# PaddlePaddle/PaddleScience

Measured on NVIDIA H100. Metric: collocation-points/sec PDE residual loss+grad (LDC N-S), higher is better.
Workload: dtype f32

## Files before the change

### paddlescience_b200/csrc/kernels_wgmma.cuh

```cuda
#pragma once

#include "kernels_thin.cuh"

#ifndef PPSCI_EMUL
#include <stdint.h>

namespace ppsci {
namespace wg {

constexpr int KCH = 32;
constexpr int THREADS = 256;
constexpr int TM = 64;
constexpr int A_TILE_BYTES = TM * KCH * 4;
__host__ __device__ inline int tile_points(int C) { return TM / C; }

__host__ __device__ inline int stage_bytes(int N) { return 2 * A_TILE_BYTES + 2 * N * KCH * 4; }
__host__ __device__ inline int fwd_smem_bytes(int N) { return 2 * stage_bytes(N) + 1024 + 64; }
constexpr int PREFETCH_MAX_CS = 8;

__host__ __device__ __forceinline__ uint32_t sw128(int row, int kk) {
  return (uint32_t)(row * 128 + ((((kk >> 2) ^ row) & 7) << 4) + ((kk & 3) << 2));
}
__device__ __forceinline__ uint32_t sw128_q(int row, int kq) { return (uint32_t)(row * 128 + (((kq ^ row) & 7) << 4)); }

__device__ __forceinline__ uint32_t smem_u32(const void* p) { return (uint32_t)__cvta_generic_to_shared(p); }

__device__ __forceinline__ float tf32_rn(float x) {
  uint32_t u;
  asm("cvt.rna.tf32.f32 %0, %1;" : "=r"(u) : "f"(x));
  return __uint_as_float(u);
}

__device__ __forceinline__ void mbar_init(uint32_t bar, uint32_t count) {
  asm volatile("mbarrier.init.shared::cta.b64 [%0], %1;" ::"r"(bar), "r"(count) : "memory");
}
__device__ __forceinline__ void mbar_expect_tx(uint32_t bar, uint32_t bytes) {
  asm volatile("mbarrier.arrive.expect_tx.shared::cta.b64 _, [%0], %1;" ::"r"(bar), "r"(bytes) : "memory");
}
__device__ __forceinline__ bool mbar_try_wait(uint32_t bar, uint32_t parity) {
  uint32_t ok;
  asm volatile(
      "{\n\t.reg .pred p;\n\t"
      "mbarrier.try_wait.parity.shared::cta.b64 p, [%1], %2;\n\t"
      "selp.u32 %0, 1, 0, p;\n\t}"
      : "=r"(ok)
      : "r"(bar), "r"(parity)
      : "memory");
  return ok != 0;
}
__device__ __forceinline__ void mbar_wait(uint32_t bar, uint32_t parity) {
  uint32_t spins = 0;
  while (!mbar_try_wait(bar, parity)) {
    if (++spins > (1u << 26)) __trap();
  }
}
__device__ __forceinline__ void bulk_g2s(uint32_t dst_smem, const void* src, uint32_t bytes, uint32_t bar) {
  asm volatile("cp.async.bulk.shared::cluster.global.mbarrier::complete_tx::bytes [%0], [%1], %2, [%3];" ::"r"(dst_smem),
               "l"(src), "r"(bytes), "r"(bar)
               : "memory");
}
__device__ __forceinline__ void fence_proxy_async() { asm volatile("fence.proxy.async.shared::cta;" ::: "memory"); }

__device__ __forceinline__ uint64_t make_desc(uint32_t saddr) {
  uint64_t d = 0;
  d |= (uint64_t)((saddr & 0x3FFFFu) >> 4);
  d |= (uint64_t)1 << 16;
  d |= (uint64_t)(1024 >> 4) << 32;
  d |= (uint64_t)1 << 62;
  return d;
}
__device__ __forceinline__ void wgmma_fence() { asm volatile("wgmma.fence.sync.aligned;" ::: "memory"); }
__device__ __forceinline__ void wgmma_commit() { asm volatile("wgmma.commit_group.sync.aligned;" ::: "memory"); }
template <int N>
__device__ __forceinline__ void wgmma_wait() {
  asm volatile("wgmma.wait_group.sync.aligned %0;" ::"n"(N) : "memory");
}
#define WG_T0 "%0, %1, %2, %3, %4, %5, %6, %7"
#define WG_T1 WG_T0 ", %8, %9, %10, %11, %12, %13, %14, %15"
#define WG_T2 WG_T1 ", %16, %17, %18, %19, %20, %21, %22, %23"
#define WG_T3 WG_T2 ", %24, %25, %26, %27, %28, %29, %30, %31"
#define WG_T4 WG_T3 ", %32, %33, %34, %35, %36, %37, %38, %39"
#define WG_T5 WG_T4 ", %40, %41, %42, %43, %44, %45, %46, %47"
#define WG_T6 WG_T5 ", %48, %49, %50, %51, %52, %53, %54, %55"
#define WG_T7 WG_T6 ", %56, %57, %58, %59, %60, %61, %62, %63"
#define WG_O8(b) "+f"(d[b]), "+f"(d[b + 1]), "+f"(d[b + 2]), "+f"(d[b + 3]), "+f"(d[b + 4]), "+f"(d[b + 5]), "+f"(d[b + 6]), "+f"(d[b + 7])
#define WG_O0 WG_O8(0)
#define WG_O1 WG_O0, WG_O8(8)
#define WG_O2 WG_O1, WG_O8(16)
#define WG_O3 WG_O2, WG_O8(24)
#define WG_O4 WG_O3, WG_O8(32)
#define WG_O5 WG_O4, WG_O8(40)
#define WG_O6 WG_O5, WG_O8(48)
#define WG_O7 WG_O6, WG_O8(56)
#define WG_MMA(M, G, IA, IB, IP)                                                                                  \
  __device__ __forceinline__ void wgmma_tf32(float (&d)[M / 2], uint64_t da, uint64_t db, uint32_t accumulate) { \
    asm volatile(                                                                                                 \
        "{\n\t.reg .pred p;\n\t"                                                                                  \
        "setp.ne.b32 p, %" #IP ", 0;\n\t"                                                                          \
        "wgmma.mma_async.sync.aligned.m64n" #M "k8.f32.tf32.tf32 {" WG_T##G "}, %" #IA ", %" #IB ", p, 1, 1;\n\t}"  \
        : WG_O##G                                                                                                 \
        : "l"(da), "l"(db), "r"(accumulate));                                                                     \
  }
WG_MMA(16, 0, 8, 9, 10)
WG_MMA(32, 1, 16, 17, 18)
WG_MMA(48, 2, 24, 25, 26)
WG_MMA(64, 3, 32, 33, 34)
WG_MMA(80, 4, 40, 41, 42)
WG_MMA(96, 5, 48, 49, 50)
WG_MMA(112, 6, 56, 57, 58)
WG_MMA(128, 7, 64, 65, 66)
#undef WG_MMA

__global__ void k_wg_prep_w(const float* __restrict__ W, float* __restrict__ img, int K, int N, int transposed) {
  const long long i = (long long)blockIdx.x * blockDim.x + threadIdx.x;
  if (i >= (long long)K * N) return;
  const int n = (int)(i / K), k = (int)(i % K);
  const float w = transposed ? W[(long long)n * K + k] : W[(long long)k * N + n];
  const float hi = tf32_rn(w);
  float* blk = img + (long long)(k / KCH) * 2 * N * KCH;
  const uint32_t off = sw128(n, k % KCH) >> 2;
  blk[off] = hi;
  blk[(long long)N * KCH + off] = w - hi;
}

struct WgArgs {
  AOperand<float> A;
  JetLayout J;
  const float* Wimg;
  int Kdim;
  int Kvalid;
  int Nout;
  const float* bias;
  float* Out;
  int ldo;
  long long oplane;
  long long Np;
  int num_tiles;
  const float* Zprev;
  int ldz;
  long long zplane;
  int act;
};

__device__ __forceinline__ unsigned char* xchg(unsigned char* base_ptr, int sbytes, int N, int r, int col) {
  return base_ptr + sbytes + 2 * A_TILE_BYTES + r * N * 4 + ((((col >> 2) ^ r) & 7) << 4) + (((col >> 2) & ~7) << 4) +
         (col & 3) * 4;
}

template <class L, int NQ, bool DX>
__global__ void __launch_bounds__(THREADS, 1) k_wg_layer(WgArgs g) {
  PPSCI_DYN_SMEM(smem_dyn);
  const uint32_t base = (smem_u32(smem_dyn) + 1023u) & ~1023u;
  unsigned char* base_ptr = smem_dyn + (base - smem_u32(smem_dyn));
  constexpr int CS = L::CS;
  constexpr int TP = TM / CS;
  constexpr int rows_used = CS * TP;
  constexpr int PPR = (THREADS / 32) * 4;
  constexpr int MAXI = (TP + PPR - 1) / PPR;
  constexpr int N = NQ * 32;
  constexpr int NH = N / 2;
  constexpr bool PREFETCH = CS <= PREFETCH_MAX_CS;
  const int sbytes = stage_bytes(N);
  const uint32_t bar0 = base + 2 * sbytes;
  const uint32_t b_bytes = (uint32_t)(2 * N * KCH * 4);
  const int tid = threadIdx.x, warp = tid >> 5, lane = tid & 31, wgi = tid >> 7;
  const int kq = lane & 7, psub = lane >> 3;
  const int nchunks = g.Kdim / KCH;
  const int act = g.A.act;

  if (tid == 0) {
    mbar_init(bar0, 1);
    mbar_init(bar0 + 8, 1);
    asm volatile("fence.mbarrier_init.release.cluster;" ::: "memory");
  }
  for (int s = 0; s < 2; ++s) {
    float4* az = reinterpret_cast<float4*>(base_ptr + s * sbytes);
    for (int i = tid; i < 2 * A_TILE_BYTES / 16; i += THREADS) az[i] = make_float4(0.f, 0.f, 0.f, 0.f);
  }
  fence_proxy_async();
  __syncthreads();

  float4 z[MAXI][CS];
  bool zok[MAXI];
  auto load_z = [&](int tile, int j) {
#pragma unroll
    for (int i = 0; i < MAXI; ++i) {
      const int pl = warp * 4 + psub + i * PPR;
      const long long p = (long long)tile * TP + pl;
      zok[i] = pl < TP && tile < g.num_tiles && p < g.Np;
      if (g.Kvalid && j * KCH + 4 * kq >= g.Kvalid) zok[i] = false;
      const float* src = g.A.Z + p * g.A.ld + j * KCH + 4 * kq;
#pragma unroll
      for (int c = 0; c < CS; ++c)
        z[i][c] = zok[i] ? __ldg(reinterpret_cast<const float4*>(src + (long long)c * g.A.plane)) : make_float4(0.f, 0.f, 0.f, 0.f);
    }
  };
  if constexpr (PREFETCH) load_z(blockIdx.x, 0);

  float ex[NH / 2], cr[NH / 2];
  const int rbase = (warp & 3) * 16 + (lane >> 2);
  const int cbase = wgi * NH + 2 * (lane & 3);
  uint32_t it = 0;
  for (int tile = blockIdx.x; tile < g.num_tiles; tile += gridDim.x) {
    const long long p0 = (long long)tile * TP;
#pragma unroll
    for (int e = 0; e < NH / 2; ++e) ex[e] = cr[e] = 0.f;
    for (int j = 0; j < nchunks; ++j, ++it) {
      const uint32_t s = it & 1u;
      wgmma_wait<1>();
      __syncthreads();
      const uint32_t st_addr = base + s * sbytes;
      unsigned char* st_ptr = base_ptr + s * sbytes;
      if (tid == 0) {
        mbar_expect_tx(bar0 + 8 * s, b_bytes);
        bulk_g2s(st_addr + 2 * A_TILE_BYTES, g.Wimg + (long long)j * 2 * N * KCH, b_bytes, bar0 + 8 * s);
      }
      if constexpr (!PREFETCH) load_z(tile, j);
#pragma unroll
      for (int i = 0; i < MAXI; ++i) {
        const int pl = warp * 4 + psub + i * PPR;
        if (pl >= TP) continue;
        const bool valid = zok[i];
        float yout[CS][4];
        if constexpr (DX) {
#pragma unroll
          for (int c = 0; c < CS; ++c) {
            yout[c][0] = z[i][c].x; yout[c][1] = z[i][c].y; yout[c][2] = z[i][c].z; yout[c][3] = z[i][c].w;
          }
        } else {
#pragma unroll
          for (int t = 0; t < 4; ++t) {
            auto comp = [&](const float4& v) { return t == 0 ? v.x : t == 1 ? v.y : t == 2 ? v.z : v.w; };
            float sc[6];
            float y0;
            act_coef<float, L::KM>(act, comp(z[i][0]), y0, sc);
            yout[0][t] = valid ? y0 : 0.f;
            jet_fwd<float, L>(g.J, sc, [&](int c) { return comp(z[i][c]); }, [&](int c, float v) { yout[c][t] = valid ? v : 0.f; });
          }
        }
#pragma unroll
        for (int c = 0; c < CS; ++c) {
          float4 h, l;
          h.x = tf32_rn(yout[c][0]); h.y = tf32_rn(yout[c][1]); h.z = tf32_rn(yout[c][2]); h.w = tf32_rn(yout[c][3]);
          l.x = yout[c][0] - h.x; l.y = yout[c][1] - h.y; l.z = yout[c][2] - h.z; l.w = yout[c][3] - h.w;
          const uint32_t off = sw128_q(c * TP + pl, kq);
          *reinterpret_cast<float4*>(st_ptr + off) = h;
          *reinterpret_cast<float4*>(st_ptr + A_TILE_BYTES + off) = l;
        }
      }
      if constexpr (PREFETCH) {
        if (j + 1 < nchunks) load_z(tile, j + 1);
        else load_z(tile + gridDim.x, 0);
      }
      fence_proxy_async();
      __syncthreads();
      mbar_wait(bar0 + 8 * s, (it >> 1) & 1u);
      const uint64_t a_hi = make_desc(st_addr), a_lo = make_desc(st_addr + A_TILE_BYTES);
      const uint64_t b_hi = make_desc(st_addr + 2 * A_TILE_BYTES + wgi * NH * 128), b_lo = b_hi + (uint64_t)(N * 128 / 16);
      wgmma_fence();
#pragma unroll
      for (int ks = 0; ks < KCH / 8; ++ks) {
        const uint64_t inc = (uint64_t)(2 * ks);
        const uint32_t first = (j == 0 && ks == 0) ? 0u : 1u;
        wgmma_tf32(ex, a_hi + inc, b_hi + inc, first);
        wgmma_tf32(cr, a_lo + inc, b_hi + inc, first);
        wgmma_tf32(cr, a_hi + inc, b_lo + inc, 1u);
      }
      wgmma_commit();
    }
    wgmma_wait<0>();
    if constexpr (!DX) {
#pragma unroll
      for (int h = 0; h < 2; ++h) {
        const int r = rbase + 8 * h;
        const int c = r / TP, pl = r - c * TP;
        const long long p = p0 + pl;
        if (r >= rows_used || p >= g.Np) continue;
        float* out_row = g.Out + (long long)c * g.oplane + p * g.ldo;
#pragma unroll
        for (int j = 0; j < NH / 8; ++j) {
          const int col = cbase + 8 * j;
          float2 v = make_float2(ex[4 * j + 2 * h] + cr[4 * j + 2 * h], ex[4 * j + 2 * h + 1] + cr[4 * j + 2 * h + 1]);
          if (c == 0 && g.bias) {
            v.x += __ldg(g.bias + col);
            v.y += __ldg(g.bias + col + 1);
          }
          *reinterpret_cast<float2*>(out_row + col) = v;
        }
      }
    } else {
      __syncthreads();
#pragma unroll
      for (int h = 0; h < 2; ++h) {
        const int r = rbase + 8 * h;
#pragma unroll
        for (int j = 0; j < NH / 8; ++j)
          *reinterpret_cast<float2*>(xchg(base_ptr, sbytes, N, r, cbase + 8 * j)) =
              make_float2(ex[4 * j + 2 * h] + cr[4 * j + 2 * h], ex[4 * j + 2 * h + 1] + cr[4 * j + 2 * h + 1]);
      }
      constexpr int N4 = N / 4;
      auto load_zc = [&](int item, float4 (&zc)[CS]) {
        const int pl = item / N4, q = item - pl * N4;
        const long long p = p0 + pl;
        if (item >= TP * N4 || p >= g.Np) return;
#pragma unroll
        for (int c = 0; c < CS; ++c)
          zc[c] = __ldg(reinterpret_cast<const float4*>(g.Zprev + (long long)c * g.zplane + p * g.ldz + 4 * q));
      };
      float4 znext[CS];
      if constexpr (PREFETCH) load_zc(tid, znext);
      __syncthreads();
      for (int item = tid; item < TP * N4; item += THREADS) {
        const int pl = item / N4, q = item - pl * N4;
        const long long p = p0 + pl;
        float4 zc[CS];
        if constexpr (PREFETCH) {
#pragma unroll
          for (int c = 0; c < CS; ++c) zc[c] = znext[c];
          load_zc(item + THREADS, znext);
        } else {
          load_zc(item, zc);
        }
        if (p >= g.Np) continue;
        float4 xc[CS];
#pragma unroll
        for (int c = 0; c < CS; ++c) xc[c] = *reinterpret_cast<const float4*>(xchg(base_ptr, sbytes, N, c * TP + pl, 4 * q));
        float ob[CS][4];
#pragma unroll
        for (int t = 0; t < 4; ++t) {
          auto comp = [&](const float4& v) { return t == 0 ? v.x : t == 1 ? v.y : t == 2 ? v.z : v.w; };
          float sc[6];
          float y0;
          act_coef<float, L::KM + 1>(g.act, comp(zc[0]), y0, sc);
          ob[0][t] = jet_adj<float, L>(g.J, sc, [&](int c) { return comp(zc[c]); }, [&](int c) { return comp(xc[c]); },
                                       [&](int c, float v) { ob[c][t] = v; });
        }
        float* out = g.Out + p * g.ldo + 4 * q;
#pragma unroll
        for (int c = 0; c < CS; ++c)
          *reinterpret_cast<float4*>(out + (long long)c * g.oplane) = make_float4(ob[c][0], ob[c][1], ob[c][2], ob[c][3]);
      }
      fence_proxy_async();
      __syncthreads();
    }
  }
}

__host__ __device__ constexpr int dw_pch(int C) { return C >= 8 ? 4 : C >= 3 ? 8 : 32 / C; }
__host__ __device__ constexpr int dw_groups(int C) { return dw_pch(C) / 4 * C; }
__host__ __device__ constexpr int dw_ksteps(int C) { return (dw_groups(C) + 1) / 2; }
__host__ __device__ constexpr int dw_atoms(int C) { return (dw_ksteps(C) + 3) / 4; }
__host__ __device__ constexpr int dw_maxq(int C) { return C <= 5 ? 4 : C <= 8 ? 2 : 1; }
__host__ __device__ constexpr int dw_smem_bytes(int C, int bnq) {
  return 2 * 2 * dw_atoms(C) * bnq * 32 * 128 + bnq * 32 * 4 + dw_pch(C) / 4 * 2 * C * 256 * 4 + bnq * 32 * 2 * 256 + 1024;
}
constexpr int DW_TK = 128;
constexpr int DW_FLUSH_ROWS = 512;
__host__ __device__ constexpr int dw_flush(int C) {
  return DW_FLUSH_ROWS / (dw_pch(C) * C) > 1 ? DW_FLUSH_ROWS / (dw_pch(C) * C) : 1;
}

struct WgDwArgs {
  AOperand<float> A;
  JetLayout J;
  const float* Zbar;
  int ldzb;
  long long zbplane;
  int Kdim;
  int Nout;
  int col_blocks;
  float* dW;
  float* db;
  long long Np;
  int chunks_per_split;
};

__device__ __forceinline__ void wgmma_tf32_rA_m64n64(float (&d)[32], const uint32_t (&a)[4], uint64_t db) {
  asm volatile(
      "{\n\t.reg .pred p;\n\t"
      "setp.ne.b32 p, %37, 0;\n\t"
      "wgmma.mma_async.sync.aligned.m64n64k8.f32.tf32.tf32 "
      "{%0, %1, %2, %3, %4, %5, %6, %7, %8, %9, %10, %11, %12, %13, %14, %15, "
      "%16, %17, %18, %19, %20, %21, %22, %23, %24, %25, %26, %27, %28, %29, %30, %31}, "
      "{%32, %33, %34, %35}, %36, p, 1, 1;\n\t}"
      : "+f"(d[0]), "+f"(d[1]), "+f"(d[2]), "+f"(d[3]), "+f"(d[4]), "+f"(d[5]), "+f"(d[6]), "+f"(d[7]), "+f"(d[8]),
        "+f"(d[9]), "+f"(d[10]), "+f"(d[11]), "+f"(d[12]), "+f"(d[13]), "+f"(d[14]), "+f"(d[15]), "+f"(d[16]),
        "+f"(d[17]), "+f"(d[18]), "+f"(d[19]), "+f"(d[20]), "+f"(d[21]), "+f"(d[22]), "+f"(d[23]), "+f"(d[24]),
        "+f"(d[25]), "+f"(d[26]), "+f"(d[27]), "+f"(d[28]), "+f"(d[29]), "+f"(d[30]), "+f"(d[31])
      : "r"(a[0]), "r"(a[1]), "r"(a[2]), "r"(a[3]), "l"(db), "r"(1u));
}
__device__ __forceinline__ void wgmma_tf32_rA_m64n32(float (&d)[16], const uint32_t (&a)[4], uint64_t db) {
  asm volatile(
      "{\n\t.reg .pred p;\n\t"
      "setp.ne.b32 p, %21, 0;\n\t"
      "wgmma.mma_async.sync.aligned.m64n32k8.f32.tf32.tf32 "
      "{%0, %1, %2, %3, %4, %5, %6, %7, %8, %9, %10, %11, %12, %13, %14, %15}, "
      "{%16, %17, %18, %19}, %20, p, 1, 1;\n\t}"
      : "+f"(d[0]), "+f"(d[1]), "+f"(d[2]), "+f"(d[3]), "+f"(d[4]), "+f"(d[5]), "+f"(d[6]), "+f"(d[7]), "+f"(d[8]),
        "+f"(d[9]), "+f"(d[10]), "+f"(d[11]), "+f"(d[12]), "+f"(d[13]), "+f"(d[14]), "+f"(d[15])
      : "r"(a[0]), "r"(a[1]), "r"(a[2]), "r"(a[3]), "l"(db), "r"(1u));
}

template <class L, int BNQ>
__global__ void __launch_bounds__(THREADS, 1) k_wg_dw(WgDwArgs g) {
  PPSCI_DYN_SMEM(smem_dyn);
  const uint32_t base = (smem_u32(smem_dyn) + 1023u) & ~1023u;
  unsigned char* base_ptr = smem_dyn + (base - smem_u32(smem_dyn));
  constexpr int CS = L::CS, PCH = dw_pch(CS), QPC = PCH / 4, G = dw_groups(CS), KS = dw_ksteps(CS), NA = dw_atoms(CS);
  constexpr int BN = BNQ * 32, NB = BNQ / 2, TAIL = BNQ & 1;
  constexpr int ATOM = BN * 128;
  constexpr int STAGE = 2 * NA * ATOM;
  constexpr int BI = (G * BN + THREADS - 1) / THREADS;
  const int tid = threadIdx.x, warp = tid >> 5, lane = tid & 31, wgi = tid >> 7, t = lane & 3;
  const int kb = blockIdx.x / g.col_blocks, n0 = (blockIdx.x - kb * g.col_blocks) * BN;
  const int Np = (int)g.Np;
  const int total_chunks = (Np + PCH - 1) / PCH;
  const int ch_begin = blockIdx.y * g.chunks_per_split;
  const int ch_end = ch_begin + g.chunks_per_split < total_chunks ? ch_begin + g.chunks_per_split : total_chunks;
  if (ch_begin >= ch_end) return;
  const int act = g.A.act;
  const int krow = kb * DW_TK + wgi * 64 + (warp & 3) * 16 + (lane >> 2);

  float* bsum = reinterpret_cast<float*>(base_ptr + 2 * STAGE);
  for (int i = tid; i < (2 * STAGE + BN * 4) / 16; i += THREADS)
    reinterpret_cast<float4*>(base_ptr)[i] = make_float4(0.f, 0.f, 0.f, 0.f);
  __syncthreads();

  float ex[NB > 0 ? NB : 1][32], ext[TAIL ? 16 : 1], cr[NB > 0 ? NB : 1][32], crt[TAIL ? 16 : 1];
#pragma unroll
  for (int nb = 0; nb < NB; ++nb)
#pragma unroll
    for (int i = 0; i < 32; ++i) ex[nb][i] = cr[nb][i] = 0.f;
#pragma unroll
  for (int i = 0; i < (TAIL ? 16 : 1); ++i) ext[i] = crt[i] = 0.f;

  auto acc_at = [&](int e) -> float {
    return e < 32 * NB ? ex[e >> 5][e & 31] + cr[e >> 5][e & 31] : ext[e - 32 * NB] + crt[e - 32 * NB];
  };
  float4* part = reinterpret_cast<float4*>(base_ptr + 2 * STAGE + BN * 4 + QPC * 2 * CS * THREADS * 4);
#pragma unroll
  for (int q = 0; q < BN / 8; ++q) part[q * THREADS + tid] = make_float4(0.f, 0.f, 0.f, 0.f);
  auto flush = [&]() {
#pragma unroll
    for (int q = 0; q < BN / 8; ++q) {
      float4 p = part[q * THREADS + tid];
      p.x += acc_at(4 * q); p.y += acc_at(4 * q + 1); p.z += acc_at(4 * q + 2); p.w += acc_at(4 * q + 3);
      part[q * THREADS + tid] = p;
    }
#pragma unroll
    for (int nb = 0; nb < NB; ++nb)
#pragma unroll
      for (int i = 0; i < 32; ++i) ex[nb][i] = cr[nb][i] = 0.f;
#pragma unroll
    for (int i = 0; i < (TAIL ? 16 : 1); ++i) ext[i] = crt[i] = 0.f;
  };

  float* za = reinterpret_cast<float*>(base_ptr + 2 * STAGE + BN * 4);
  auto za_at = [&](int qq, int h, int c) -> float* { return za + ((qq * 2 + h) * CS + c) * THREADS + tid; };
  float4 zb[BI];
  auto load_a = [&](int ch) {
    const int p0 = ch * PCH;
#pragma unroll
    for (int qq = 0; qq < QPC; ++qq)
#pragma unroll
      for (int h = 0; h < 2; ++h) {
        const int p = p0 + 4 * qq + t;
        const int k = krow + 8 * h;
        const bool ok = p < Np && k < g.Kdim;
        const float* src = g.A.Z + (ok ? (long long)p * g.A.ld + k : 0);
#pragma unroll
        for (int c = 0; c < CS; ++c)
          asm volatile("cp.async.ca.shared.global [%0], [%1], 4, %2;" ::"r"(smem_u32(za_at(qq, h, c))),
                       "l"(src + (ok ? (long long)c * g.A.plane : 0)), "r"(ok ? 4 : 0)
                       : "memory");
      }
    asm volatile("cp.async.commit_group;" ::: "memory");
  };
  auto load_b = [&](int ch) {
    const int p0 = ch * PCH;
#pragma unroll
    for (int i = 0; i < BI; ++i) {
      const int item = tid + THREADS * i;
      const int gi = item / BN, n = item - gi * BN;
      const int qq = gi / CS, c = gi - qq * CS;
      const int p = p0 + 4 * qq;
      const bool ok = item < G * BN && n0 + n < g.Nout;
      const float* src = g.Zbar + (long long)c * g.zbplane + (long long)p * g.ldzb + n0 + n;
      zb[i].x = ok && p < Np ? __ldg(src) : 0.f;
      zb[i].y = ok && p + 1 < Np ? __ldg(src + g.ldzb) : 0.f;
      zb[i].z = ok && p + 2 < Np ? __ldg(src + 2 * g.ldzb) : 0.f;
      zb[i].w = ok && p + 3 < Np ? __ldg(src + 3 * g.ldzb) : 0.f;
    }
  };

  load_a(ch_begin);
  load_b(ch_begin);
  uint32_t ahi[KS][4], alo[KS][4];
  for (int ch = ch_begin; ch < ch_end; ++ch) {
    const int sidx = (ch - ch_begin) & 1;
    const uint32_t st_addr = base + sidx * STAGE;
    unsigned char* st = base_ptr + sidx * STAGE;
#pragma unroll
    for (int i = 0; i < BI; ++i) {
      const int item = tid + THREADS * i;
      if (item >= G * BN) continue;
      const int gi = item / BN, n = item - gi * BN;
      const float4 v = zb[i];
      float4 hi, lo;
      hi.x = tf32_rn(v.x); hi.y = tf32_rn(v.y); hi.z = tf32_rn(v.z); hi.w = tf32_rn(v.w);
      lo.x = v.x - hi.x; lo.y = v.y - hi.y; lo.z = v.z - hi.z; lo.w = v.w - hi.w;
      const uint32_t off = (gi >> 3) * ATOM + sw128_q(n, gi & 7);
      *reinterpret_cast<float4*>(st + off) = hi;
      *reinterpret_cast<float4*>(st + NA * ATOM + off) = lo;
      if (kb == 0 && gi % CS == 0) atomicAdd(bsum + n, (v.x + v.y) + (v.z + v.w));
    }
    wgmma_wait<0>();
    if (ch > ch_begin && (ch - ch_begin) % dw_flush(CS) == 0) flush();
    asm volatile("cp.async.wait_group 0;" ::: "memory");
    float av[QPC][2][CS];
#pragma unroll
    for (int qq = 0; qq < QPC; ++qq)
#pragma unroll
      for (int h = 0; h < 2; ++h) {
        float z[CS], sc[6];
#pragma unroll
        for (int c = 0; c < CS; ++c) z[c] = *za_at(qq, h, c);
        act_coef<float, L::KM>(act, z[0], av[qq][h][0], sc);
        jet_fwd<float, L>(g.J, sc, [&](int c) { return z[c]; }, [&](int c, float v) { av[qq][h][c] = v; });
      }
    if (ch + 1 < ch_end) load_a(ch + 1);
    fence_proxy_async();
    __syncthreads();
    if (ch + 1 < ch_end) load_b(ch + 1);
#pragma unroll
    for (int s = 0; s < KS; ++s)
#pragma unroll
      for (int e = 0; e < 2; ++e)
#pragma unroll
        for (int h = 0; h < 2; ++h) {
          const int gi = 2 * s + e;
          const float v = gi < G ? av[gi / CS][h][gi % CS] : 0.f;
          const float vh = tf32_rn(v);
          ahi[s][2 * e + h] = __float_as_uint(vh);
          alo[s][2 * e + h] = __float_as_uint(v - vh);
        }
    wgmma_fence();
#pragma unroll
    for (int s = 0; s < KS; ++s) {
      const uint64_t b_hi = make_desc(st_addr + (s >> 2) * ATOM + (s & 3) * 32);
      const uint64_t b_lo = b_hi + (uint64_t)(NA * ATOM / 16);
#pragma unroll
      for (int nb = 0; nb < NB; ++nb) {
        const uint64_t bo = (uint64_t)(nb * 64 * 128 / 16);
        wgmma_tf32_rA_m64n64(ex[nb], ahi[s], b_hi + bo);
        wgmma_tf32_rA_m64n64(cr[nb], alo[s], b_hi + bo);
        wgmma_tf32_rA_m64n64(cr[nb], ahi[s], b_lo + bo);
      }
      if constexpr (TAIL) {
        const uint64_t bo = (uint64_t)(NB * 64 * 128 / 16);
        wgmma_tf32_rA_m64n32(ext, ahi[s], b_hi + bo);
        wgmma_tf32_rA_m64n32(crt, alo[s], b_hi + bo);
        wgmma_tf32_rA_m64n32(crt, ahi[s], b_lo + bo);
      }
    }
    wgmma_commit();
  }
  wgmma_wait<0>();
#pragma unroll
  for (int h = 0; h < 2; ++h) {
    const int k = krow + 8 * h;
    if (k >= g.Kdim) continue;
    float* row = g.dW + (long long)k * g.Nout + n0;
#pragma unroll
    for (int j = 0; j < BN / 8; ++j) {
      if (n0 + 8 * j >= g.Nout) break;
      const int col = 8 * j + 2 * t;
      const float4 p = part[j * THREADS + tid];
      atomicAdd(row + col, (h ? p.z : p.x) + acc_at(4 * j + 2 * h));
      atomicAdd(row + col + 1, (h ? p.w : p.y) + acc_at(4 * j + 2 * h + 1));
    }
  }
  if (kb == 0) {
    __syncthreads();
    if (tid < BN && n0 + tid < g.Nout) atomicAdd(g.db + n0 + tid, bsum[tid]);
  }
}

}

inline int wg_kpad(int K) { return (K + wg::KCH - 1) / wg::KCH * wg::KCH; }
inline bool wg_shape_ok(int K, int N) { return K % wg::KCH == 0 && K >= 32 && K <= 1024 && N % 32 == 0 && N >= 32 && N <= 256; }
inline bool wg_plan_ok(const ppsci_plan_spec& s, const JetLayout& J) {
  return s.dtype == PPSCI_F32 && !s.gated && !act_has_param(s.act) && with_lay(WgLays{}, J, [](auto) {});
}
inline bool wg_fwd_ok(const ppsci_plan_spec& s, int l) {
  if (l == 1) return s.dense_in && s.n_layers >= 2 && s.widths[0] % 4 == 0 && wg_shape_ok(wg_kpad(s.widths[0]), s.widths[1]);
  if (l < 2 || l > s.n_layers) return false;
  return wg_shape_ok(s.widths[l - 1], s.widths[l]);
}
inline bool wg_dx_ok(const ppsci_plan_spec& s, int l) {
  if (l < 2 || l > s.n_layers) return false;
  return wg_shape_ok(s.widths[l], s.widths[l - 1]);
}

inline bool wg_dw_ok(const ppsci_plan_spec& s, int l) {
  if (l < 1 || (l == 1 && !s.dense_in) || l > s.n_layers) return false;
  const int K = s.widths[l - 1], N = s.widths[l];
  return K % 4 == 0 && N % 32 == 0 && N >= 32 && N <= 256;
}

}
#endif
```

Before: 6.042 million.

## Decouple weight B-tile staging into a 3-stage ring prefetched one chunk ahead

Splits the shared-memory stages so the A tiles stay double-buffered while the weight (B) tiles move to a separate three-slot ring with their own mbarriers. Each iteration issues the bulk copy for the next chunk (or the next tile's first chunk) ahead of time, so the weight load overlaps the current chunk's A-tile construction and wgmma instead of being issued and waited on in the same iteration. The DX exchange buffer is moved onto the last-used B slot. This uses more shared memory and adds some ring-indexing complexity, with a risk of slot-reuse hazards at tile boundaries.

```diff
diff --git a/paddlescience_b200/csrc/kernels_wgmma.cuh b/paddlescience_b200/csrc/kernels_wgmma.cuh
--- a/paddlescience_b200/csrc/kernels_wgmma.cuh
+++ b/paddlescience_b200/csrc/kernels_wgmma.cuh
@@ -14,8 +14,10 @@
 constexpr int A_TILE_BYTES = TM * KCH * 4;
 __host__ __device__ inline int tile_points(int C) { return TM / C; }
 
-__host__ __device__ inline int stage_bytes(int N) { return 2 * A_TILE_BYTES + 2 * N * KCH * 4; }
-__host__ __device__ inline int fwd_smem_bytes(int N) { return 2 * stage_bytes(N) + 1024 + 64; }
+constexpr int A_STAGE_BYTES = 2 * A_TILE_BYTES;
+constexpr int B_STAGES = 3;
+__host__ __device__ inline int b_stage_bytes(int N) { return 2 * N * KCH * 4; }
+__host__ __device__ inline int fwd_smem_bytes(int N) { return 2 * A_STAGE_BYTES + B_STAGES * b_stage_bytes(N) + 1024 + 64; }
 constexpr int PREFETCH_MAX_CS = 8;
 
 __host__ __device__ __forceinline__ uint32_t sw128(int row, int kk) {
@@ -142,9 +144,8 @@
   int act;
 };
 
-__device__ __forceinline__ unsigned char* xchg(unsigned char* base_ptr, int sbytes, int N, int r, int col) {
-  return base_ptr + sbytes + 2 * A_TILE_BYTES + r * N * 4 + ((((col >> 2) ^ r) & 7) << 4) + (((col >> 2) & ~7) << 4) +
-         (col & 3) * 4;
+__device__ __forceinline__ unsigned char* xchg(unsigned char* xb, int N, int r, int col) {
+  return xb + r * N * 4 + ((((col >> 2) ^ r) & 7) << 4) + (((col >> 2) & ~7) << 4) + (col & 3) * 4;
 }
 
 template <class L, int NQ, bool DX>
@@ -160,22 +161,21 @@
   constexpr int N = NQ * 32;
   constexpr int NH = N / 2;
   constexpr bool PREFETCH = CS <= PREFETCH_MAX_CS;
-  const int sbytes = stage_bytes(N);
-  const uint32_t bar0 = base + 2 * sbytes;
-  const uint32_t b_bytes = (uint32_t)(2 * N * KCH * 4);
+  const uint32_t b_bytes = (uint32_t)b_stage_bytes(N);
+  const uint32_t b_base = base + 2 * A_STAGE_BYTES;
+  const uint32_t bar0 = b_base + B_STAGES * b_bytes;
   const int tid = threadIdx.x, warp = tid >> 5, lane = tid & 31, wgi = tid >> 7;
   const int kq = lane & 7, psub = lane >> 3;
   const int nchunks = g.Kdim / KCH;
   const int act = g.A.act;
 
   if (tid == 0) {
-    mbar_init(bar0, 1);
-    mbar_init(bar0 + 8, 1);
+    for (int b = 0; b < B_STAGES; ++b) mbar_init(bar0 + 8 * b, 1);
     asm volatile("fence.mbarrier_init.release.cluster;" ::: "memory");
   }
   for (int s = 0; s < 2; ++s) {
-    float4* az = reinterpret_cast<float4*>(base_ptr + s * sbytes);
-    for (int i = tid; i < 2 * A_TILE_BYTES / 16; i += THREADS) az[i] = make_float4(0.f, 0.f, 0.f, 0.f);
+    float4* az = reinterpret_cast<float4*>(base_ptr + s * A_STAGE_BYTES);
+    for (int i = tid; i < A_STAGE_BYTES / 16; i += THREADS) az[i] = make_float4(0.f, 0.f, 0.f, 0.f);
   }
   fence_proxy_async();
   __syncthreads();
@@ -200,21 +200,24 @@
   float ex[NH / 2], cr[NH / 2];
   const int rbase = (warp & 3) * 16 + (lane >> 2);
   const int cbase = wgi * NH + 2 * (lane & 3);
+  auto fetch_w = [&](int j, uint32_t b) {
+    mbar_expect_tx(bar0 + 8 * b, b_bytes);
+    bulk_g2s(b_base + b * b_bytes, g.Wimg + (long long)j * 2 * N * KCH, b_bytes, bar0 + 8 * b);
+  };
+  if (tid == 0) fetch_w(0, 0);
   uint32_t it = 0;
   for (int tile = blockIdx.x; tile < g.num_tiles; tile += gridDim.x) {
     const long long p0 = (long long)tile * TP;
 #pragma unroll
     for (int e = 0; e < NH / 2; ++e) ex[e] = cr[e] = 0.f;
     for (int j = 0; j < nchunks; ++j, ++it) {
-      const uint32_t s = it & 1u;
+      const uint32_t s = it & 1u, bs = it % B_STAGES;
       wgmma_wait<1>();
       __syncthreads();
-      const uint32_t st_addr = base + s * sbytes;
-      unsigned char* st_ptr = base_ptr + s * sbytes;
-      if (tid == 0) {
-        mbar_expect_tx(bar0 + 8 * s, b_bytes);
-        bulk_g2s(st_addr + 2 * A_TILE_BYTES, g.Wimg + (long long)j * 2 * N * KCH, b_bytes, bar0 + 8 * s);
-      }
+      const uint32_t st_addr = base + s * A_STAGE_BYTES;
+      unsigned char* st_ptr = base_ptr + s * A_STAGE_BYTES;
+      if (tid == 0 && (j + 1 < nchunks || tile + (int)gridDim.x < g.num_tiles))
+        fetch_w(j + 1 < nchunks ? j + 1 : 0, bs == B_STAGES - 1 ? 0 : bs + 1);
       if constexpr (!PREFETCH) load_z(tile, j);
 #pragma unroll
       for (int i = 0; i < MAXI; ++i) {
@@ -254,9 +257,9 @@
       }
       fence_proxy_async();
       __syncthreads();
-      mbar_wait(bar0 + 8 * s, (it >> 1) & 1u);
+      mbar_wait(bar0 + 8 * bs, (it / B_STAGES) & 1u);
       const uint64_t a_hi = make_desc(st_addr), a_lo = make_desc(st_addr + A_TILE_BYTES);
-      const uint64_t b_hi = make_desc(st_addr + 2 * A_TILE_BYTES + wgi * NH * 128), b_lo = b_hi + (uint64_t)(N * 128 / 16);
+      const uint64_t b_hi = make_desc(b_base + bs * b_bytes + wgi * NH * 128), b_lo = b_hi + (uint64_t)(N * 128 / 16);
       wgmma_fence();
 #pragma unroll
       for (int ks = 0; ks < KCH / 8; ++ks) {
@@ -290,12 +293,13 @@
       }
     } else {
       __syncthreads();
+      unsigned char* xb = base_ptr + 2 * A_STAGE_BYTES + ((it - 1) % B_STAGES) * b_bytes;
 #pragma unroll
       for (int h = 0; h < 2; ++h) {
         const int r = rbase + 8 * h;
 #pragma unroll
         for (int j = 0; j < NH / 8; ++j)
-          *reinterpret_cast<float2*>(xchg(base_ptr, sbytes, N, r, cbase + 8 * j)) =
+          *reinterpret_cast<float2*>(xchg(xb, N, r, cbase + 8 * j)) =
               make_float2(ex[4 * j + 2 * h] + cr[4 * j + 2 * h], ex[4 * j + 2 * h + 1] + cr[4 * j + 2 * h + 1]);
       }
       constexpr int N4 = N / 4;
@@ -324,7 +328,7 @@
         if (p >= g.Np) continue;
         float4 xc[CS];
 #pragma unroll
-        for (int c = 0; c < CS; ++c) xc[c] = *reinterpret_cast<const float4*>(xchg(base_ptr, sbytes, N, c * TP + pl, 4 * q));
+        for (int c = 0; c < CS; ++c) xc[c] = *reinterpret_cast<const float4*>(xchg(xb, N, c * TP + pl, 4 * q));
         float ob[CS][4];
 #pragma unroll
         for (int t = 0; t < 4; ++t) {
```

After: 6.112 million (median of 6 runs). 1.2% higher.
